# JunzheJosephZhu/DenseMatcher

Measured on AMD Instinct MI355X. Metric: mesh-pairs/sec at N=2048 D=768 k=128, higher is better.
Workload: dtype f16; 1 GPU; configs[1]: batch=64 pairs, N=2048, D=768, k=128 functional-map solve; pairs_per_gpu=64, N=2048, D=768, k=128, basis_dtype=float64, parallelism=pairs sharded over 1 GPU(s), one process per GPU, no data-path collective, process_group_size=1

## Files before the change

### densematcher_amd/csrc/dm_ctx.hip

```cpp
#include <stdarg.h>

#include "dm_internal.h"

int dm_fail(dm_ctx* ctx, int code, const char* fmt, ...) {
    char buf[1024];
    va_list ap;
    va_start(ap, fmt);
    vsnprintf(buf, sizeof(buf), fmt, ap);
    va_end(ap);
    if (ctx) ctx->err = buf;
    return code;
}

static thread_local std::string g_create_err = "null context";

static int create_fail(const char* what, hipError_t e) {
    char buf[512];
    snprintf(buf, sizeof(buf), "dm_create: %s%s%s", what, e != hipSuccess ? ": " : "", e != hipSuccess ? hipGetErrorString(e) : "");
    g_create_err = buf;
    return DM_EHIP;
}

extern "C" int dm_create(int device, void* hip_stream, dm_ctx** out) {
    if (!out) return DM_EINVAL;
// ... 60 lines not shown
    else if (n == "simnn_prio") ctx->opt_simnn_prio = value;
    else if (n == "fit_mfma") ctx->opt_fit_mfma = value;
    else if (n == "solve_pcg") ctx->opt_solve_pcg = value;
    else if (n == "basis_stats") { ctx->opt_basis_stats = value; for (auto& e : ctx->stats) e.valid = false; }
    else if (n == "lsa_reg") ctx->opt_lsa_reg = value;
    else if (n == "p2p_split") ctx->opt_p2p_split = value;
    else if (n == "simnn_persist") ctx->opt_simnn_persist = value;
    else if (n == "p2pfm_direct") ctx->opt_p2pfm_direct = value;
    else if (n == "zoomout_fused") ctx->opt_zoomout_fused = value;
    else if (n == "simnn1_wt") ctx->opt_simnn1_wt = value;
    else if (n == "zoomout_sub_fused") ctx->opt_zoomout_sub_fused = value;
    else if (n == "fps_heat_route") ctx->opt_fps_heat_route = value;
    else if (n == "graph_geod_device") ctx->opt_graph_geod_device = value;
    else if (n == "fmn_eig_route") ctx->opt_fmn_eig_route = value;
    else if (n == "proj_onepass") ctx->opt_proj_onepass = value;
    else return dm_fail(ctx, DM_EINVAL, "dm_set_option: unknown option '%s'", name);
    return DM_OK;
}

extern "C" const char* dm_last_error(const dm_ctx* ctx) { return ctx ? ctx->err.c_str() : g_create_err.c_str(); }
extern "C" const char* dm_version(void) { return DM_VERSION_STRING; }
extern "C" size_t dm_workspace_bytes(const dm_ctx* ctx) { return ctx ? ctx->ws_bytes : 0; }

dm_ctx::basis_stat* dm_stat_entry(dm_ctx* ctx, const void* ptr, int B, int N, int k, int ld, int esz, int n) {
    for (auto& e : ctx->stats)
        if (e.ptr == ptr && e.B == B && e.N == N && e.k == k && e.ld == ld && e.esz == esz && e.n == n && e.buf[0]) return &e;
    dm_ctx::basis_stat& e = ctx->stats[ctx->stats_next];
    ctx->stats_next = (ctx->stats_next + 1) % 4;
    const size_t need = (size_t)B * n * 8;
    if (!e.buf[0] || (size_t)e.B * e.n * 8 < need) {
// ... 131 lines not shown
```

### densematcher_amd/csrc/dm_fmap.hip

```cpp
#include <stdlib.h>

#include "dm_gemm_f64.h"
#include "dm_internal.h"
#include "dm_pcg.h"

struct OutProj {
    float* direct;
    double* partial;
    int B, k, D;
    __device__ __forceinline__ void store(int b, int split, int m, int c, double v) const {
        if (direct) direct[((long long)b * k + m) * D + c] = (float)v;
        else partial[(((long long)split * B + b) * k + m) * D + c] = v;
    }
};

__global__ __launch_bounds__(256) void splitk_reduce_f32_kernel(const double* __restrict__ partial, int nsplit,
                                                                long long n, float* __restrict__ out) {
    const long long i = (long long)blockIdx.x * 256 + threadIdx.x;
    if (i >= n) return;
    double s = 0.0;
    for (int q = 0; q < nsplit; ++q) s += partial[(long long)q * n + i];
    out[i] = (float)s;
}

// ... 887 lines not shown
    DM_REQUIRE(ctx, w_descr >= 0.0 && w_lap >= 0.0 && (w_descr > 0.0 || w_lap > 0.0), "weights must be >= 0 and not both 0");
    DM_CHECK_HIP(ctx, hipSetDevice(ctx->device));
    const size_t bA = (size_t)B * k1 * D * 4, bB = (size_t)B * k2 * D * 4;
    const fmap_solve_plan plan = fmap_solve_plan_for(ctx, B, k1, k2);
    int rc = dm_ws_reserve(ctx, dm_project_f16split_ws(B, N1, D, k1, ld1, (int)sizeof(TR)) + dm_project_f16split_ws(B, N2, D, k2, ld2, (int)sizeof(TR)) +
                                    dm_align_up(bA) + dm_align_up(bB) + dm_align_up((size_t)B * 8) + fmap_solve_ws(plan) + 8192);
    if (rc) return rc;
    double* c00 = (double*)dm_ws_take(ctx, (size_t)B * 8);
    if (!c00) return dm_fail(ctx, DM_ENOMEM, "fmap_fit: workspace not reserved");
    const bool lazy = dm_cdiv(N1, 1024) <= 2 && dm_cdiv(N2, 1024) <= 2;
    float* A = lazy ? nullptr : (float*)dm_ws_take(ctx, bA);
    float* Bm = lazy ? nullptr : (float*)dm_ws_take(ctx, bB);
    if (!lazy && (!A || !Bm)) return dm_fail(ctx, DM_ENOMEM, "fmap_fit: workspace not reserved");
    const float* pA = nullptr; const float* pB = nullptr;
    int nsA = 1, nsB = 1;
    rc = dm_project_f16split_launch<TR>(ctx, B, N1, D, k1, Phi1, ld1, mass1, F1, A, &pA, &nsA);
    if (rc) return rc;
    const dm_c00_args<TR> cz{Phi1, (long long)N1 * ld1, Phi2, (long long)N2 * ld2, mass1, mass2, N1, N2, c00};
    rc = dm_project_f16split_launch<TR>(ctx, B, N2, D, k2, Phi2, ld2, mass2, F2, Bm, &pB, &nsB, &cz);
    if (rc) return rc;
    if (lazy) {
        const long long sA = nsA == 2 ? (long long)B * k1 * D : 0, sB = nsB == 2 ? (long long)B * k2 * D : 0;
        KRowsStackedPart opa{pA, pB, sA, sB, k1, k2, D};
        KRowsPart opb{pA, sA, k1, D};
        return fmap_solve_core(ctx, plan, B, k1, k2, D, opa, opb, lam1, lam2, c00, w_descr, w_lap, C, info);
    }
    KRowsStackedF32 opa{A, Bm, k1, k2, D};
    KRowsF32 opb{A, (long long)k1 * D, D, k1, D};
    return fmap_solve_core(ctx, plan, B, k1, k2, D, opa, opb, lam1, lam2, c00, w_descr, w_lap, C, info);
}
extern "C" int dm_fmap_fit(dm_ctx* ctx, int B, int N1, int N2, int D, int k1, int k2, const float* Phi1, int ld1, const float* Phi2,
                           int ld2, const float* mass1, const float* mass2, const void* F1, const void* F2, const double* lam1,
                           const double* lam2, double w_descr, double w_lap, double* C, int32_t* info) {
    return fmap_fit_impl<float>(ctx, B, N1, N2, D, k1, k2, Phi1, ld1, Phi2, ld2, mass1, mass2, F1, F2, lam1, lam2, w_descr, w_lap, C, info);
// ... 7 lines not shown
```

### densematcher_amd/csrc/dm_internal.h

```cpp
#pragma once

#include <hip/hip_runtime.h>
#include <stdint.h>
#include <stdio.h>
#include <string.h>

#include <string>
#include <unordered_map>
#include <vector>

#include "densematch.h"

#define DM_VERSION_STRING "densematch 0.5.0 (gfx950, abi 7)"

struct dm_ctx {
    int device = 0;
    hipStream_t stream = nullptr;
    std::string err;

    char* ws = nullptr;
    size_t ws_bytes = 0;
    size_t ws_off = 0;

    std::string prof_name;
    std::vector<hipEvent_t> prof_events;
    std::vector<const char*> prof_names;
    std::vector<const char*> prof_syms;
    size_t prof_used = 0;

    std::unordered_map<const void*, size_t> lds_granted;

    int opt_simnn_pipe = 1;
    int opt_knn_split = 1;
    int opt_solve_packed = 0;
    int opt_proj_onepass = 1;
    int opt_fit_mfma = 1;
    int opt_simnn_prio = 0;
    int opt_simnn_big = 0;
    int opt_simnn_band = 4;
    int opt_lsa_reg = 2;
    int opt_solve_pcg = 1;
    int opt_solve_reg = 1;
    int opt_p2p_split = 2;
    int opt_simnn_persist = 1;
    int opt_p2pfm_direct = 1;
    int opt_simnn1_wt = 4;
    int opt_zoomout_fused = 1;
    int opt_zoomout_sub_fused = 1;
    int opt_fps_heat_route = 0;
    int opt_graph_geod_device = 1;
// ... 211 lines not shown
                             int ld2, const float* mass1, const float* A, const float* Bm, const double* lam1, const double* lam2,
                             const double* ops1, const double* ops2, int n_ops, const double* weights, const double* C, double* energy,
                             double* grad, double* keep, bool keep_valid);

int dm_eig_jacobi_sorted(dm_ctx* ctx, int B, int m, double* H, double* V, double* theta, double* Q);

size_t lsa_ws_bytes(int B, int nr, int nc);
int lsa_run(dm_ctx* ctx, int B, int nr, int nc, const double* dense, int n_lr, int KP, const double* E2p, const double* P1p,
            const double* a1p, int maximize, int32_t* col_of_row, int32_t* info);

size_t dm_project_f16split_ws(int B, int N, int D, int k, int ld, int real_bytes);
template <typename TR>
int dm_project_f16split_launch(dm_ctx* ctx, int B, int N, int D, int k, const TR* Phi, int ld, const TR* mass, const void* F,
                               float* Ared, const float** partial_out, int* nsplit_out, const dm_c00_args<TR>* cz = nullptr);
template <typename TR>
int dm_project_f16split(dm_ctx* ctx, int B, int N, int D, int k, const TR* Phi, int ld, const TR* mass,
                        const void* F, float* Ared);
```

### densematcher_amd/csrc/dm_project.hip

```cpp
#include "dm_device.h"
#include "dm_internal.h"

typedef unsigned int u32x4 __attribute__((ext_vector_type(4)));
typedef __fp16 h4_t __attribute__((__vector_size__(4 * sizeof(__fp16))));

constexpr int PT = 128;
constexpr int PTD = 192;
constexpr int PNT = PTD / 64;
constexpr int PFV = PTD / 64;
constexpr int PBK = 32;
constexpr int PLD = 160;
constexpr int PLDF = 224;
constexpr int PSTAGE = 2 * PBK * PLD + PBK * PLDF;

template <int LD>
__device__ __forceinline__ f16x8 tr_frag(const _Float16* base, int row0, int col, int lane) {
    const int t = lane & 15;
    const _Float16* p = base + (row0 + (t >> 2)) * LD + col + 4 * (t & 3);
    const h4_t a = __builtin_amdgcn_ds_read_tr16_b64_v4f16((__attribute__((address_space(3))) h4_t*)p);
    const h4_t b = __builtin_amdgcn_ds_read_tr16_b64_v4f16((__attribute__((address_space(3))) h4_t*)(p + 4 * LD));
    f16x8 r;
    r[0] = (_Float16)a[0]; r[1] = (_Float16)a[1]; r[2] = (_Float16)a[2]; r[3] = (_Float16)a[3];
    r[4] = (_Float16)b[0]; r[5] = (_Float16)b[1]; r[6] = (_Float16)b[2]; r[7] = (_Float16)b[3];
    return r;
// ... 230 lines not shown
        for (int nt = 0; nt < PNT; ++nt)
#pragma unroll
            for (int r = 0; r < 16; ++r) {
                const int m = m0 + wm * 64 + mt * 32 + (r & 3) + 8 * (r >> 2) + 4 * (lane >> 5);
                const int d = d0 + wn * (PTD / 2) + nt * 32 + (lane & 31);
                if (m < p.k && d < p.D) out[(long long)m * p.D + d] = acc[mt][nt][r] * inv_scale;
            }
}

constexpr int P2TD = 384;
constexpr int P2NT = 3;
constexpr int P2LDF = 416;
constexpr int P2STAGE = 2 * PBK * PLD + PBK * P2LDF;
constexpr size_t P2_LDS = (size_t)2 * P2STAGE * sizeof(_Float16) + 16;

template <typename TR>
struct proj2_params {
    const TR* Phi; const TR* mass; const _Float16* F;
    float* partial;
    int B, N, D, k, ld, nsplit, kchunk, tiles_m, tiles_d, ntiles;
    dm_c00_args<TR> cz; int with_c00;
    int flip;
};

template <typename TR, int NMT>
__device__ __forceinline__ void proj2_body(const proj2_params<TR>& p, _Float16* smem, unsigned* slot, int b, int split, int m0, int d0) {
    const int t = threadIdx.x, lane = t & 63, wave = t >> 6;
    const int wm = wave >> 2, wn = wave & 3;
    const int nbeg = split * p.kchunk, nend = min(p.N, nbeg + p.kchunk);
    const TR* Phi = p.Phi + (long long)b * p.N * p.ld;
    const TR* mass = p.mass + (long long)b * p.N;
    const _Float16* F = p.F + (long long)b * p.N * p.D;

    f32x16 acc[NMT > 0 ? NMT : 1][P2NT];
#pragma unroll
    for (int a = 0; a < (NMT > 0 ? NMT : 1); ++a)
#pragma unroll
        for (int c = 0; c < P2NT; ++c)
#pragma unroll
            for (int r = 0; r < 16; ++r) acc[a][c][r] = 0.f;

    const int srow = t >> 4, scol = (t & 15) * 8;
    const int fcol = (t & 15) * (P2TD / 16);
    typedef int i32x4_t __attribute__((ext_vector_type(4)));
    constexpr int NQ = (int)sizeof(TR) / 2;
    const __amdgpu_buffer_rsrc_t rX = __builtin_amdgcn_make_buffer_rsrc(const_cast<TR*>(Phi), (short)0, (int)((unsigned)p.N * p.ld * sizeof(TR)), 0x00020000);
    const __amdgpu_buffer_rsrc_t rM = __builtin_amdgcn_make_buffer_rsrc(const_cast<TR*>(mass), (short)0, (int)((unsigned)p.N * sizeof(TR)), 0x00020000);
    const __amdgpu_buffer_rsrc_t rF = __builtin_amdgcn_make_buffer_rsrc(const_cast<_Float16*>(F), (short)0, (int)((unsigned)p.N * p.D * 2), 0x00020000);
    unsigned colmask = 0;
#pragma unroll
    for (int q = 0; q < 8; ++q) colmask |= (m0 + scol + q < p.k) ? (1u << q) : 0u;
    i32x4_t xrA[NQ], xrB[NQ], anA, anB;
    float xf[8];
    i32x4_t frA[3], frB[3];
#define P2_FENCE() { asm volatile("" ::: "memory"); __builtin_amdgcn_sched_barrier(0); }
#define P2_FETCH_X(s_, xr, an_raw)                                                                            \
    {                                                                                                         \
        const int n_ = nbeg + (s_) * PBK + srow;                                                              \
        const int vo = colmask ? (n_ * p.ld + m0 + scol) * (int)sizeof(TR) : 0x7fffff00;    \
        _Pragma("unroll") for (int q = 0; q < NQ; ++q) xr[q] = __builtin_amdgcn_raw_buffer_load_b128(rX, vo + 16 * q, 0, 0);   \
        if constexpr (sizeof(TR) == 8) {                                                                      \
            const auto m2 = __builtin_amdgcn_raw_buffer_load_b64(rM, n_ * 8, 0, 0);                           \
            an_raw[0] = m2[0]; an_raw[1] = m2[1];                                                             \
        } else {                                                                                              \
            an_raw[0] = __builtin_amdgcn_raw_buffer_load_b32(rM, n_ * 4, 0, 0);                               \
        }                                                                                                     \
        P2_FENCE()                                                                                            \
    }
#define P2_FETCH_F(s_, fr)                                                                                    \
    {                                                                                                         \
        const int n_ = nbeg + (s_) * PBK + srow;                                                              \
        const int vo = (n_ * p.D + d0 + fcol) * 2;                                                            \
        _Pragma("unroll") for (int q = 0; q < 3; ++q) fr[q] = __builtin_amdgcn_raw_buffer_load_b128(rF, vo + 16 * q, 0, 0);   \
        P2_FENCE()                                                                                            \
    }
#define P2_PUBLISH(s_, xr, an_raw)                                                                            \
    {                                                                                                         \
        const bool rv = nbeg + (s_) * PBK + srow < nend;                                                      \
        float an;                                                                                             \
        if constexpr (sizeof(TR) == 8) an = (float)__hiloint2double(an_raw[1], an_raw[0]);                    \
        else an = __int_as_float(an_raw[0]);                                                                  \
        an = rv ? an : 0.f;                                 \
        float mx = 0.f;                                                                                       \
        _Pragma("unroll") for (int q = 0; q < 8; ++q) {                                                       \
            float x_;                                                                                         \
            if constexpr (sizeof(TR) == 8) x_ = (float)__hiloint2double(xr[q >> 1][2 * (q & 1) + 1], xr[q >> 1][2 * (q & 1)]);   \
            else x_ = __int_as_float(xr[q >> 2][q & 3]);                                                      \
            float v_ = x_ * an;                                                                               \
            asm volatile("" : "+v"(v_));                                                                      \
            xf[q] = v_;                                                                                       \
        }                                                                                                     \
        if (colmask != 0xffu && colmask != 0u) {      \
            _Pragma("unroll") for (int q = 0; q < 8; ++q) xf[q] = ((colmask >> q) & 1u) ? xf[q] : 0.f;    \
        }                                                                                                     \
        _Pragma("unroll") for (int q = 0; q < 8; ++q) mx = fmaxf(mx, fabsf(xf[q]));                           \
             \
        mx = fmaxf(mx, __builtin_bit_cast(float, __builtin_amdgcn_update_dpp(0, __builtin_bit_cast(int, mx), 0xB1, 0xF, 0xF, true)));   \
        mx = fmaxf(mx, __builtin_bit_cast(float, __builtin_amdgcn_update_dpp(0, __builtin_bit_cast(int, mx), 0x4E, 0xF, 0xF, true)));   \
        mx = fmaxf(mx, __builtin_bit_cast(float, __builtin_amdgcn_update_dpp(0, __builtin_bit_cast(int, mx), 0x141, 0xF, 0xF, true)));  \
        mx = fmaxf(mx, __builtin_bit_cast(float, __builtin_amdgcn_update_dpp(0, __builtin_bit_cast(int, mx), 0x140, 0xF, 0xF, true)));  \
        const unsigned mu = __builtin_bit_cast(unsigned, mx);                                                 \
        const unsigned m01 = max((unsigned)__builtin_amdgcn_readlane((int)mu, 0), (unsigned)__builtin_amdgcn_readlane((int)mu, 16));   \
        const unsigned m23 = max((unsigned)__builtin_amdgcn_readlane((int)mu, 32), (unsigned)__builtin_amdgcn_readlane((int)mu, 48));  \
        const unsigned mw = max(m01, m23);                                                                    \
        if (lane == 0 && mw != 0u) __hip_atomic_fetch_max(&slot[(s_) % 3], mw, __ATOMIC_RELAXED, __HIP_MEMORY_SCOPE_WORKGROUP);        \
    }
#define P2_STASH(s_, buf_, fr)                                                                                   \
    {                                                                                                         \
        const float smx = __builtin_bit_cast(float, slot[(s_) % 3]);                                          \
        if (smx > run_max) {                                                                                  \
            run_max = smx;                                                                                    \
            int ex = 0;                                                                                       \
            (void)frexpf(smx, &ex);                                                                           \
            const int e2 = min(14 - ex, 100);                                                                 \
            if (e2 < cur_e) {            \
                ratio = ldexpf(1.0f, e2 - cur_e);                                                             \
                cur_e = e2;                                                                                   \
                scale = ldexpf(1.0f, e2);                                                                     \
            }                                                                                                 \
        }                                                                                                     \
        _Float16* Xh = smem + (buf_) * P2STAGE + srow * PLD + scol;                                           \
        _Float16* Xl = Xh + PBK * PLD;                                                                        \
        _Float16* Fs = smem + (buf_) * P2STAGE + 2 * PBK * PLD + srow * P2LDF + fcol;                         \
        f16x8 h, l;                                                                                           \
// ... 7 lines not shown
        *reinterpret_cast<f16x8*>(Xl) = l;                                                                    \
        const bool rvf = nbeg + (s_) * PBK + srow < nend;                                                     \
        _Pragma("unroll") for (int q = 0; q < 3; ++q)                                                         \
            *reinterpret_cast<i32x4_t*>(Fs + 8 * q) = rvf ? fr[q] : i32x4_t{0, 0, 0, 0};                      \
    }

#define P2_RESCALE()                                                                                          \
    if (ratio != 1.0f) {                                                                                      \
        _Pragma("unroll") for (int a = 0; a < (NMT > 0 ? NMT : 1); ++a)                                       \
            _Pragma("unroll") for (int c = 0; c < P2NT; ++c)                                                  \
                _Pragma("unroll") for (int r = 0; r < 16; ++r) acc[a][c][r] *= ratio;                         \
        ratio = 1.0f;                                                                                         \
    }
    float run_max = 0.f, scale = ldexpf(1.0f, 100), ratio = 1.0f;
    int cur_e = 100;
    const int ns = (nend - nbeg + PBK - 1) / PBK;
    if (t < 3) slot[t] = 0u;
    __syncthreads();
    if (ns > 0) {
        P2_FETCH_X(0, xrA, anA)
        P2_FETCH_F(0, frA)
        P2_FETCH_X(1, xrB, anB)
        P2_FETCH_F(1, frB)
        P2_PUBLISH(0, xrA, anA)
        P2_FETCH_X(2, xrA, anA)
    }
    __syncthreads();
    if (ns > 0) {
        P2_STASH(0, 0, frA)
        ratio = 1.0f;
        if (ns > 1) P2_PUBLISH(1, xrB, anB)
    }
    __syncthreads();
#define P2_MMA(buf_)                                                                                          \
        if constexpr (NMT > 0) {                                                                              \
            const _Float16* Xh = smem + (buf_) * P2STAGE;                                                     \
            const _Float16* Xl = Xh + PBK * PLD;                                                              \
            const _Float16* Fs = Xl + PBK * PLD;                                                              \
            _Pragma("unroll") for (int ks = 0; ks < PBK / 16; ++ks) {                                         \
                const int row0 = ks * 16 + 8 * (lane >> 5);                                                   \
                const int sub = 16 * ((lane >> 4) & 1);                \
                f16x8 ah[NMT > 0 ? NMT : 1], al[NMT > 0 ? NMT : 1], bf[P2NT];                                 \
                _Pragma("unroll") for (int x = 0; x < NMT; ++x) {                                             \
                    ah[x] = tr_frag<PLD>(Xh, row0, wm * 64 + x * 32 + sub, lane);                             \
                    al[x] = tr_frag<PLD>(Xl, row0, wm * 64 + x * 32 + sub, lane);                             \
                }                                                                                             \
                _Pragma("unroll") for (int x = 0; x < P2NT; ++x)                                              \
                    bf[x] = tr_frag<P2LDF>(Fs, row0, wn * (P2TD / 4) + x * 32 + sub, lane);                   \
                _Pragma("unroll") for (int mt = 0; mt < NMT; ++mt)                                            \
                    _Pragma("unroll") for (int nt = 0; nt < P2NT; ++nt) {                                     \
                        acc[mt][nt] = __builtin_amdgcn_mfma_f32_32x32x16_f16(ah[mt], bf[nt], acc[mt][nt], 0, 0, 0);   \
                        acc[mt][nt] = __builtin_amdgcn_mfma_f32_32x32x16_f16(al[mt], bf[nt], acc[mt][nt], 0, 0, 0);   \
                    }                                                                                         \
            }                                                                                                 \
        }
#define P2_ITER(s_, XL, ANL, XU, ANU, FL, FU)                                                                 \
    {                                                                                                         \
        const int buf = (s_) & 1;                                                                             \
        P2_FETCH_X((s_) + 3, XL, ANL)                                         \
        P2_FETCH_F((s_) + 2, FL)                                                                              \
        if (p.flip && wave >= 4) {                                                                            \
            if ((s_) + 1 < ns) { P2_STASH((s_) + 1, buf ^ 1, FU) }                                            \
            if ((s_) + 2 < ns) { P2_PUBLISH((s_) + 2, XU, ANU) }                                              \
            __builtin_amdgcn_sched_barrier(0);                                                                \
            P2_MMA(buf)                                                                                       \
        } else {                                                                                              \
            P2_MMA(buf)                                                                                       \
            __builtin_amdgcn_sched_barrier(0);                                                                \
            if ((s_) + 1 < ns) { P2_STASH((s_) + 1, buf ^ 1, FU) }                                            \
            if ((s_) + 2 < ns) { P2_PUBLISH((s_) + 2, XU, ANU) }                                              \
        }                                                                                                     \
        P2_RESCALE()                                                                                          \
        if (t == 0) slot[(s_) % 3] = 0u;                      \
        __syncthreads();                                                                                      \
    }
    for (int s = 0; s < ns; s += 2) {
        P2_ITER(s, xrB, anB, xrA, anA, frA, frB)
        if (s + 1 < ns) P2_ITER(s + 1, xrA, anA, xrB, anB, frB, frA)
    }
#undef P2_ITER
#undef P2_FENCE
#undef P2_MMA
#undef P2_RESCALE
#undef P2_FETCH_X
#undef P2_FETCH_F
#undef P2_PUBLISH
#undef P2_STASH

    if constexpr (NMT > 0) {
        const float inv_scale = 1.0f / scale;
        float* out = p.partial + ((long long)split * p.B + b) * p.k * p.D;
#pragma unroll
        for (int mt = 0; mt < NMT; ++mt)
#pragma unroll
            for (int nt = 0; nt < P2NT; ++nt)
#pragma unroll
                for (int r = 0; r < 16; ++r) {
                    const int m = m0 + wm * 64 + mt * 32 + (r & 3) + 8 * (r >> 2) + 4 * (lane >> 5);
                    const int d = d0 + wn * (P2TD / 4) + nt * 32 + (lane & 31);
                    if (m < p.k && d < p.D) out[(long long)m * p.D + d] = acc[mt][nt][r] * inv_scale;
                }
    }
}

template <typename TR>
__global__ __launch_bounds__(512, 2) void proj_onepass_kernel(proj2_params<TR> p) {
    extern __shared__ __attribute__((aligned(16))) _Float16 smem[];
    const int t = threadIdx.x;
    if ((int)blockIdx.x >= p.ntiles) {
        __shared__ double red[2][4];
        dm_c00_body<TR>(p.cz, (int)blockIdx.x - p.ntiles, t, red);
        return;
    }
    unsigned* slot = reinterpret_cast<unsigned*>(smem + 2 * P2STAGE);
    const int ntile = p.tiles_m * p.tiles_d;
    const int id = xcd_remap(blockIdx.x, p.ntiles);
    const int tile = id % ntile;
    const int split = (id / ntile) % p.nsplit;
    const int b = id / (ntile * p.nsplit);
    const int tm = tile / p.tiles_d, td = tile - tm * p.tiles_d;
    const int m0 = tm * PT, d0 = td * P2TD;
    const int wm = __builtin_amdgcn_readfirstlane(t >> 8);
    const int left = p.k - (m0 + wm * 64);
    if (left > 32) proj2_body<TR, 2>(p, smem, slot, b, split, m0, d0);
    else if (left > 0) proj2_body<TR, 1>(p, smem, slot, b, split, m0, d0);
    else proj2_body<TR, 0>(p, smem, slot, b, split, m0, d0);
}

__global__ __launch_bounds__(256) void proj_reduce_kernel(const float* __restrict__ partial, int nsplit, long long n,
                                                          float* __restrict__ out) {
    const long long i = (long long)blockIdx.x * 256 + threadIdx.x;
    if (i >= n) return;
    double s = 0.0;
    for (int q = 0; q < nsplit; ++q) s += (double)partial[(long long)q * n + i];
    out[i] = (float)s;
}

size_t dm_project_f16split_ws(int B, int N, int D, int k, int ld, int real_bytes) {
    const int nsplit = dm_cdiv(N, 1024);
    return dm_align_up((size_t)nsplit * B * k * D * 4) + dm_align_up((size_t)B * 64 * 4) + 4096 +
           (real_bytes == 8 ? dm_align_up((size_t)B * N * ld * 4) + dm_align_up((size_t)B * N * 4) : 0);
}

template <typename TR>
int dm_project_f16split_launch(dm_ctx* ctx, int B, int N, int D, int k, const TR* Phi, int ld, const TR* mass,
                               const void* F, float* Ared, const float** partial_out, int* nsplit_out, const dm_c00_args<TR>* cz) {
    proj_params<TR> p;
    p.Phi = Phi; p.mass = mass; p.F = (const _Float16*)F;
    p.B = B; p.N = N; p.D = D; p.k = k; p.ld = ld;
    p.tiles_m = dm_cdiv(k, PT); p.tiles_d = dm_cdiv(D, PTD);
    p.kchunk = 1024;
    const int nsplit = dm_cdiv(N, p.kchunk);
    p.nsplit = nsplit;
    if ((long long)N * ld >= (1ll << 31)) return dm_fail(ctx, DM_EINVAL, "dm_project: N * ld must be below 2^31");
    const size_t pbytes = (size_t)nsplit * B * k * D * 4;
    int rc = DM_OK;
    p.partial = (float*)dm_ws_take(ctx, pbytes);
    const int n_part = max(1, min(64, (int)(((long long)N * ld) / 4096)));
    float* amax_part = (float*)dm_ws_take(ctx, (size_t)B * n_part * 4);
    if (!p.partial || !amax_part) return dm_fail(ctx, DM_ENOMEM, "dm_project: workspace not reserved");
    p.amax_part = amax_part; p.n_part = n_part;
    const size_t lds = (size_t)2 * PSTAGE * sizeof(_Float16);
    const bool onepass_ok = (long long)N * ld * (long long)sizeof(TR) < (1ll << 31) - 4096 && (long long)N * D * 2 < (1ll << 31) && (D & 1) == 0 &&
                            (((uintptr_t)F) & 3) == 0;
    if (ctx->opt_proj_onepass && onepass_ok) {
        proj2_params<TR> q;
        q.Phi = Phi; q.mass = mass; q.F = p.F; q.partial = p.partial;
        q.B = B; q.N = N; q.D = D; q.k = k; q.ld = ld; q.nsplit = nsplit; q.kchunk = p.kchunk;
        q.tiles_m = p.tiles_m; q.tiles_d = dm_cdiv(D, P2TD); q.ntiles = q.tiles_m * q.tiles_d * nsplit * B;
        q.with_c00 = cz ? 1 : 0;
        q.flip = 1;
#ifdef DM_EXPERIMENTS
        q.flip = dm_knob("DM_PROJ_FLIP", 1);
#endif
        q.cz = cz ? *cz : dm_c00_args<TR>{};
        rc = dm_grant_lds(ctx, (const void*)proj_onepass_kernel<TR>, P2_LDS);
        if (rc) return rc;
        DM_LAUNCH(ctx, "project_f16split_mfma", proj_onepass_kernel<TR>, dim3(q.ntiles + (cz ? B : 0)), dim3(512), P2_LDS, q);
    } else
    if constexpr (sizeof(TR) == 8) {
        float* phi32 = (float*)dm_ws_take(ctx, (size_t)B * N * ld * 4);
        float* mass32 = (float*)dm_ws_take(ctx, (size_t)B * N * 4);
        if (!phi32 || !mass32) return dm_fail(ctx, DM_ENOMEM, "dm_project: workspace not reserved");
        DM_LAUNCH(ctx, "project_absmax", proj_absmax_kernel<TR>, dim3(n_part + (cz ? 1 : 0), B), dim3(256), 0, Phi, mass, N, ld, k, amax_part, phi32,
                  mass32, n_part, cz ? *cz : dm_c00_args<TR>{});
        proj_params<float> pf;
        pf.Phi = phi32; pf.mass = mass32; pf.F = p.F; pf.amax_part = p.amax_part; pf.n_part = p.n_part; pf.partial = p.partial;
        pf.B = B; pf.N = N; pf.D = D; pf.k = k; pf.ld = ld; pf.nsplit = p.nsplit; pf.kchunk = p.kchunk; pf.tiles_m = p.tiles_m; pf.tiles_d = p.tiles_d;
        rc = dm_grant_lds(ctx, (const void*)proj_f16split_kernel<float>, lds);
        if (rc) return rc;
        DM_LAUNCH(ctx, "project_f16split_mfma", proj_f16split_kernel<float>, dim3(p.tiles_m * p.tiles_d * nsplit * B), dim3(256), lds, pf);
    } else {
        DM_LAUNCH(ctx, "project_absmax", proj_absmax_kernel<TR>, dim3(n_part + (cz ? 1 : 0), B), dim3(256), 0, Phi, mass, N, ld, k, amax_part,
// ... 4 lines not shown
    }
    if (partial_out) *partial_out = p.partial;
    if (nsplit_out) *nsplit_out = nsplit;
    if (Ared) {
        const long long n = (long long)B * k * D;
        DM_LAUNCH(ctx, "project_reduce", proj_reduce_kernel, dim3((unsigned)((n + 255) / 256)), dim3(256), 0, p.partial, nsplit, n,
                  Ared);
    }
    return DM_OK;
}
template int dm_project_f16split_launch<float>(dm_ctx*, int, int, int, int, const float*, int, const float*, const void*, float*, const float**, int*,
                                               const dm_c00_args<float>*);
template int dm_project_f16split_launch<double>(dm_ctx*, int, int, int, int, const double*, int, const double*, const void*, float*, const float**, int*,
                                                const dm_c00_args<double>*);

template <typename TR>
int dm_project_f16split(dm_ctx* ctx, int B, int N, int D, int k, const TR* Phi, int ld, const TR* mass,
                        const void* F, float* Ared) {
    int rc = dm_ws_reserve(ctx, dm_project_f16split_ws(B, N, D, k, ld, (int)sizeof(TR)));
    if (rc) return rc;
    return dm_project_f16split_launch<TR>(ctx, B, N, D, k, Phi, ld, mass, F, Ared, nullptr, nullptr, nullptr);
}
template int dm_project_f16split<float>(dm_ctx*, int, int, int, int, const float*, int, const float*, const void*, float*);
template int dm_project_f16split<double>(dm_ctx*, int, int, int, int, const double*, int, const double*, const void*, float*);
```

### densematcher_amd/engine.py

```python
import ctypes as C
import types

import numpy as np
import torch

from . import _lib
from ._engine_aggre import _AggreOps
from ._engine_dnet import _DiffusionNetOps
from ._engine_eval import _EvalOps
from ._engine_geodesic import GraphTooWide, _GeodesicOps, heat_geodesic_check
from ._engine_jbu import _JbuOps
from ._engine_lift import _LiftOps
from ._engine_mesh import _MeshOps
from ._engine_network import _NetworkOps
from ._engine_render import _RenderOps
from ._engine_vit import _VitOps
from ._operands import fits_abi, host_ptr, ptr as _ptr


class MatchEngine(_MeshOps, _GeodesicOps, _DiffusionNetOps, _LiftOps, _RenderOps, _JbuOps, _AggreOps, _VitOps, _EvalOps, _NetworkOps):
    def __init__(self, device=None, lib_path=None):
        if not torch.cuda.is_available():
            raise RuntimeError("MatchEngine needs a ROCm GPU (gfx950); there is no CPU fallback")
        self.lib = _lib.load(lib_path)
# ... 64 lines not shown
            raise ValueError("matrix contains invalid numeric entries")
        if worst == 1:
            raise ValueError("cost matrix is infeasible")

    def _reals(self, *arrays):
        def dt(a):
            return a.dtype if isinstance(a, torch.Tensor) else getattr(a, "dtype", None)
        f64 = any(a is not None and str(dt(a)).endswith("float64") for a in arrays)
        tdt = torch.float64 if f64 else torch.float32
        return ("_f64" if f64 else "",) + tuple(None if a is None else self._dev(a, tdt, "real") for a in arrays)

    def synchronize(self):
        self.stream.synchronize()

    OPTION_DEFAULTS = {"simnn_pipe": 1, "simnn_persist": 1, "knn_split": 1, "p2p_split": 2, "solve_packed": 0, "solve_reg": 1, "simnn_band": 4, "lsa_reg": 2, "simnn_big": 0,
                       "p2pfm_direct": 1, "zoomout_fused": 1, "proj_onepass": 1, "fit_mfma": 1, "basis_stats": 1, "solve_pcg": 1,
                       "zoomout_sub_fused": 1, "fps_heat_route": 0, "graph_geod_device": 1, "fmn_eig_route": 0}

    def set_option(self, name, value):
        self._chk(self.lib.dm_set_option(self.ctx, name.encode(), int(value)))
        self._options[name] = int(value)

    def get_option(self, name):
        return self._options[name]

    def reset_options(self):
        for k, v in self.OPTION_DEFAULTS.items():
            self.set_option(k, v)

    @staticmethod
    def split_depth(k):
# ... 578 lines not shown
```

Before: 62080 mesh-pairs/s.

## Fuse both mesh projections into one persistent pipelined kernel with cross-tile prefetch

Replaces the two separate one-pass projection launches, one per mesh, with a single persistent kernel sized to the CU count. It walks tiles from both meshes and prefetches the next tile's first stages while the current tile's tail is still computing. This is meant to remove a kernel launch, the tail idle at tile boundaries, and the extra c00 blocks. The price is more register pressure from carrying prefetch state, more complex slot and ring indexing, and a fixed grid that may load-balance worse.

After: 62580 mesh-pairs/s (median of 6 runs). No clear change (+0.8%).

```diff
diff --git a/densematcher_amd/csrc/dm_ctx.hip b/densematcher_amd/csrc/dm_ctx.hip
--- a/densematcher_amd/csrc/dm_ctx.hip
+++ b/densematcher_amd/csrc/dm_ctx.hip
@@ -98,6 +98,7 @@
     else if (n == "graph_geod_device") ctx->opt_graph_geod_device = value;
     else if (n == "fmn_eig_route") ctx->opt_fmn_eig_route = value;
     else if (n == "proj_onepass") ctx->opt_proj_onepass = value;
+    else if (n == "proj_pipeline") ctx->opt_proj_pipeline = value;
     else return dm_fail(ctx, DM_EINVAL, "dm_set_option: unknown option '%s'", name);
     return DM_OK;
 }
diff --git a/densematcher_amd/csrc/dm_fmap.hip b/densematcher_amd/csrc/dm_fmap.hip
--- a/densematcher_amd/csrc/dm_fmap.hip
+++ b/densematcher_amd/csrc/dm_fmap.hip
@@ -925,10 +925,8 @@
     if (!lazy && (!A || !Bm)) return dm_fail(ctx, DM_ENOMEM, "fmap_fit: workspace not reserved");
     const float* pA = nullptr; const float* pB = nullptr;
     int nsA = 1, nsB = 1;
-    rc = dm_project_f16split_launch<TR>(ctx, B, N1, D, k1, Phi1, ld1, mass1, F1, A, &pA, &nsA);
-    if (rc) return rc;
     const dm_c00_args<TR> cz{Phi1, (long long)N1 * ld1, Phi2, (long long)N2 * ld2, mass1, mass2, N1, N2, c00};
-    rc = dm_project_f16split_launch<TR>(ctx, B, N2, D, k2, Phi2, ld2, mass2, F2, Bm, &pB, &nsB, &cz);
+    rc = dm_project_pair_f16split_launch<TR>(ctx, B, D, N1, k1, Phi1, ld1, mass1, F1, A, &pA, &nsA, N2, k2, Phi2, ld2, mass2, F2, Bm, &pB, &nsB, &cz);
     if (rc) return rc;
     if (lazy) {
         const long long sA = nsA == 2 ? (long long)B * k1 * D : 0, sB = nsB == 2 ? (long long)B * k2 * D : 0;
diff --git a/densematcher_amd/csrc/dm_internal.h b/densematcher_amd/csrc/dm_internal.h
--- a/densematcher_amd/csrc/dm_internal.h
+++ b/densematcher_amd/csrc/dm_internal.h
@@ -34,6 +34,7 @@
     int opt_knn_split = 1;
     int opt_solve_packed = 0;
     int opt_proj_onepass = 1;
+    int opt_proj_pipeline = 1;
     int opt_fit_mfma = 1;
     int opt_simnn_prio = 0;
     int opt_simnn_big = 0;
@@ -275,5 +276,9 @@
 int dm_project_f16split_launch(dm_ctx* ctx, int B, int N, int D, int k, const TR* Phi, int ld, const TR* mass, const void* F,
                                float* Ared, const float** partial_out, int* nsplit_out, const dm_c00_args<TR>* cz = nullptr);
 template <typename TR>
+int dm_project_pair_f16split_launch(dm_ctx* ctx, int B, int D, int N1, int k1, const TR* Phi1, int ld1, const TR* mass1, const void* F1, float* Ared1,
+                                    const float** partial1, int* nsplit1, int N2, int k2, const TR* Phi2, int ld2, const TR* mass2, const void* F2,
+                                    float* Ared2, const float** partial2, int* nsplit2, const dm_c00_args<TR>* cz);
+template <typename TR>
 int dm_project_f16split(dm_ctx* ctx, int B, int N, int D, int k, const TR* Phi, int ld, const TR* mass,
                         const void* F, float* Ared);
diff --git a/densematcher_amd/csrc/dm_project.hip b/densematcher_amd/csrc/dm_project.hip
--- a/densematcher_amd/csrc/dm_project.hip
+++ b/densematcher_amd/csrc/dm_project.hip
@@ -268,23 +268,84 @@
 constexpr int P2STAGE = 2 * PBK * PLD + PBK * P2LDF;
 constexpr size_t P2_LDS = (size_t)2 * P2STAGE * sizeof(_Float16) + 16;
 
-template <typename TR>
-struct proj2_params {
+typedef int i32x4_t __attribute__((ext_vector_type(4)));
+
+template <typename TR>
+struct proj2_mesh {
     const TR* Phi; const TR* mass; const _Float16* F;
     float* partial;
-    int B, N, D, k, ld, nsplit, kchunk, tiles_m, tiles_d, ntiles;
+    int N, k, ld, nsplit, tiles_m, tiles_d, ntiles;
+};
+
+template <typename TR>
+struct proj2_params {
+    proj2_mesh<TR> m[2];
+    int B, D, kchunk;
+    int total;
     dm_c00_args<TR> cz; int with_c00;
     int flip;
 };
 
-template <typename TR, int NMT>
-__device__ __forceinline__ void proj2_body(const proj2_params<TR>& p, _Float16* smem, unsigned* slot, int b, int split, int m0, int d0) {
+struct proj2_tile {
+    __amdgpu_buffer_rsrc_t rX, rM, rF;
+    float* out;
+    int nbeg, nend, ns, k, ld, m0, d0;
+};
+struct proj2_src {
+    __amdgpu_buffer_rsrc_t rX, rM, rF;
+    int nbeg, nend, ld, xcol, fcol;
+    unsigned colmask;
+};
+template <typename TR>
+struct proj2_regs {
+    i32x4_t xrA[sizeof(TR) / 2], xrB[sizeof(TR) / 2], anA, anB, frA[3], frB[3];
+    float xf[8];
+};
+
+template <typename TR>
+__device__ __forceinline__ proj2_tile proj2_tile_at(const proj2_params<TR>& p, const proj2_mesh<TR> q, int id) {
+    const int ntile = q.tiles_m * q.tiles_d;
+    const int tile = id % ntile;
+    const int split = (id / ntile) % q.nsplit;
+    const int b = id / (ntile * q.nsplit);
+    const int tm = tile / q.tiles_d, td = tile - tm * q.tiles_d;
+    const TR* Phi = q.Phi + (long long)b * q.N * q.ld;
+    const TR* mass = q.mass + (long long)b * q.N;
+    const _Float16* F = q.F + (long long)b * q.N * p.D;
+    proj2_tile c;
+    c.rX = __builtin_amdgcn_make_buffer_rsrc(const_cast<TR*>(Phi), (short)0, (int)((unsigned)q.N * q.ld * sizeof(TR)), 0x00020000);
+    c.rM = __builtin_amdgcn_make_buffer_rsrc(const_cast<TR*>(mass), (short)0, (int)((unsigned)q.N * sizeof(TR)), 0x00020000);
+    c.rF = __builtin_amdgcn_make_buffer_rsrc(const_cast<_Float16*>(F), (short)0, (int)((unsigned)q.N * p.D * 2), 0x00020000);
+    c.out = q.partial + ((long long)split * p.B + b) * q.k * p.D;
+    c.nbeg = split * p.kchunk;
+    c.nend = min(q.N, c.nbeg + p.kchunk);
+    c.ns = (c.nend - c.nbeg + PBK - 1) / PBK;
+    c.k = q.k; c.ld = q.ld; c.m0 = tm * PT; c.d0 = td * P2TD;
+    return c;
+}
+__device__ __forceinline__ proj2_src proj2_src_of(const proj2_tile& c, int scol, int fcol) {
+    proj2_src s;
+    s.rX = c.rX; s.rM = c.rM; s.rF = c.rF;
+    s.nbeg = c.nbeg; s.nend = c.nend; s.ld = c.ld; s.xcol = c.m0 + scol; s.fcol = c.d0 + fcol;
+    s.colmask = 0;
+#pragma unroll
+    for (int q = 0; q < 8; ++q) s.colmask |= (s.xcol + q < c.k) ? (1u << q) : 0u;
+    return s;
+}
+__device__ __forceinline__ proj2_src proj2_pick(bool first, const proj2_src& a, const proj2_src& b) {
+    proj2_src s;
+    s.rX = first ? a.rX : b.rX; s.rM = first ? a.rM : b.rM; s.rF = first ? a.rF : b.rF;
+    s.nbeg = first ? a.nbeg : b.nbeg; s.nend = first ? a.nend : b.nend; s.ld = first ? a.ld : b.ld;
+    s.xcol = first ? a.xcol : b.xcol; s.fcol = first ? a.fcol : b.fcol; s.colmask = first ? a.colmask : b.colmask;
+    return s;
+}
+
+template <typename TR, int NMT, bool CHAIN>
+__device__ __forceinline__ void proj2_body(const proj2_tile& cur, const proj2_tile& nxt, bool chain, bool primed, int sb, int D, int flip,
+                                           proj2_regs<TR>& rg, _Float16* smem, unsigned* slot) {
     const int t = threadIdx.x, lane = t & 63, wave = t >> 6;
     const int wm = wave >> 2, wn = wave & 3;
-    const int nbeg = split * p.kchunk, nend = min(p.N, nbeg + p.kchunk);
-    const TR* Phi = p.Phi + (long long)b * p.N * p.ld;
-    const TR* mass = p.mass + (long long)b * p.N;
-    const _Float16* F = p.F + (long long)b * p.N * p.D;
+    const int nbeg = cur.nbeg, nend = cur.nend, m0 = cur.m0, d0 = cur.d0;
 
     f32x16 acc[NMT > 0 ? NMT : 1][P2NT];
 #pragma unroll
@@ -296,41 +357,35 @@
 
     const int srow = t >> 4, scol = (t & 15) * 8;
     const int fcol = (t & 15) * (P2TD / 16);
-    typedef int i32x4_t __attribute__((ext_vector_type(4)));
     constexpr int NQ = (int)sizeof(TR) / 2;
-    const __amdgpu_buffer_rsrc_t rX = __builtin_amdgcn_make_buffer_rsrc(const_cast<TR*>(Phi), (short)0, (int)((unsigned)p.N * p.ld * sizeof(TR)), 0x00020000);
-    const __amdgpu_buffer_rsrc_t rM = __builtin_amdgcn_make_buffer_rsrc(const_cast<TR*>(mass), (short)0, (int)((unsigned)p.N * sizeof(TR)), 0x00020000);
-    const __amdgpu_buffer_rsrc_t rF = __builtin_amdgcn_make_buffer_rsrc(const_cast<_Float16*>(F), (short)0, (int)((unsigned)p.N * p.D * 2), 0x00020000);
-    unsigned colmask = 0;
-#pragma unroll
-    for (int q = 0; q < 8; ++q) colmask |= (m0 + scol + q < p.k) ? (1u << q) : 0u;
-    i32x4_t xrA[NQ], xrB[NQ], anA, anB;
-    float xf[8];
-    i32x4_t frA[3], frB[3];
+    const proj2_src cs = proj2_src_of(cur, scol, fcol);
+    const proj2_src nsrc = CHAIN ? proj2_src_of(nxt, scol, fcol) : cs;
+    float (&xf)[8] = rg.xf;
 #define P2_FENCE() { asm volatile("" ::: "memory"); __builtin_amdgcn_sched_barrier(0); }
-#define P2_FETCH_X(s_, xr, an_raw)                                                                            \
+#define P2_FETCH_X(S_, s_, xr, an_raw)                                                                        \
     {                                                                                                         \
-        const int n_ = nbeg + (s_) * PBK + srow;                                                              \
-        const int vo = colmask ? (n_ * p.ld + m0 + scol) * (int)sizeof(TR) : 0x7fffff00;    \
-        _Pragma("unroll") for (int q = 0; q < NQ; ++q) xr[q] = __builtin_amdgcn_raw_buffer_load_b128(rX, vo + 16 * q, 0, 0);   \
+        const int n_ = S_.nbeg + (s_) * PBK + srow;                                                           \
+        const int vo = S_.colmask ? (n_ * S_.ld + S_.xcol) * (int)sizeof(TR) : 0x7fffff00;    \
+        _Pragma("unroll") for (int q = 0; q < NQ; ++q) xr[q] = __builtin_amdgcn_raw_buffer_load_b128(S_.rX, vo + 16 * q, 0, 0);   \
         if constexpr (sizeof(TR) == 8) {                                                                      \
-            const auto m2 = __builtin_amdgcn_raw_buffer_load_b64(rM, n_ * 8, 0, 0);                           \
+            const auto m2 = __builtin_amdgcn_raw_buffer_load_b64(S_.rM, n_ * 8, 0, 0);                        \
             an_raw[0] = m2[0]; an_raw[1] = m2[1];                                                             \
         } else {                                                                                              \
-            an_raw[0] = __builtin_amdgcn_raw_buffer_load_b32(rM, n_ * 4, 0, 0);                               \
+            an_raw[0] = __builtin_amdgcn_raw_buffer_load_b32(S_.rM, n_ * 4, 0, 0);                            \
         }                                                                                                     \
         P2_FENCE()                                                                                            \
     }
-#define P2_FETCH_F(s_, fr)                                                                                    \
+#define P2_FETCH_F(S_, s_, fr)                                                                                \
     {                                                                                                         \
-        const int n_ = nbeg + (s_) * PBK + srow;                                                              \
-        const int vo = (n_ * p.D + d0 + fcol) * 2;                                                            \
-        _Pragma("unroll") for (int q = 0; q < 3; ++q) fr[q] = __builtin_amdgcn_raw_buffer_load_b128(rF, vo + 16 * q, 0, 0);   \
+        const int n_ = S_.nbeg + (s_) * PBK + srow;                                                           \
+        const int vo = (n_ * D + S_.fcol) * 2;                                                                \
+        _Pragma("unroll") for (int q = 0; q < 3; ++q) fr[q] = __builtin_amdgcn_raw_buffer_load_b128(S_.rF, vo + 16 * q, 0, 0);   \
         P2_FENCE()                                                                                            \
     }
-#define P2_PUBLISH(s_, xr, an_raw)                                                                            \
+#define P2_PUBLISH(S_, s_, slot_, xr, an_raw)                                                                 \
     {                                                                                                         \
-        const bool rv = nbeg + (s_) * PBK + srow < nend;                                                      \
+        const unsigned colmask = S_.colmask;                                                                  \
+        const bool rv = S_.nbeg + (s_) * PBK + srow < S_.nend;                                                \
         float an;                                                                                             \
         if constexpr (sizeof(TR) == 8) an = (float)__hiloint2double(an_raw[1], an_raw[0]);                    \
         else an = __int_as_float(an_raw[0]);                                                                  \
@@ -357,11 +412,11 @@
         const unsigned m01 = max((unsigned)__builtin_amdgcn_readlane((int)mu, 0), (unsigned)__builtin_amdgcn_readlane((int)mu, 16));   \
         const unsigned m23 = max((unsigned)__builtin_amdgcn_readlane((int)mu, 32), (unsigned)__builtin_amdgcn_readlane((int)mu, 48));  \
         const unsigned mw = max(m01, m23);                                                                    \
-        if (lane == 0 && mw != 0u) __hip_atomic_fetch_max(&slot[(s_) % 3], mw, __ATOMIC_RELAXED, __HIP_MEMORY_SCOPE_WORKGROUP);        \
+        if (lane == 0 && mw != 0u) __hip_atomic_fetch_max(&slot[slot_], mw, __ATOMIC_RELAXED, __HIP_MEMORY_SCOPE_WORKGROUP);        \
     }
 #define P2_STASH(s_, buf_, fr)                                                                                   \
     {                                                                                                         \
-        const float smx = __builtin_bit_cast(float, slot[(s_) % 3]);                                          \
+        const float smx = __builtin_bit_cast(float, slot[(sb + (s_)) % 3]);                                   \
         if (smx > run_max) {                                                                                  \
             run_max = smx;                                                                                    \
             int ex = 0;                                                                                       \
@@ -399,22 +454,24 @@
     }
     float run_max = 0.f, scale = ldexpf(1.0f, 100), ratio = 1.0f;
     int cur_e = 100;
-    const int ns = (nend - nbeg + PBK - 1) / PBK;
-    if (t < 3) slot[t] = 0u;
+    const int ns = cur.ns;
+    if (!(CHAIN && primed)) {
+        if (t < 3) slot[t] = 0u;
+        __syncthreads();
+        if (ns > 0) {
+            P2_FETCH_X(cs, 0, rg.xrA, rg.anA)
+            P2_FETCH_F(cs, 0, rg.frA)
+            P2_FETCH_X(cs, 1, rg.xrB, rg.anB)
+            P2_FETCH_F(cs, 1, rg.frB)
+            P2_PUBLISH(cs, 0, sb % 3, rg.xrA, rg.anA)
+            P2_FETCH_X(cs, 2, rg.xrA, rg.anA)
+        }
+    }
     __syncthreads();
     if (ns > 0) {
-        P2_FETCH_X(0, xrA, anA)
-        P2_FETCH_F(0, frA)
-        P2_FETCH_X(1, xrB, anB)
-        P2_FETCH_F(1, frB)
-        P2_PUBLISH(0, xrA, anA)
-        P2_FETCH_X(2, xrA, anA)
-    }
-    __syncthreads();
-    if (ns > 0) {
-        P2_STASH(0, 0, frA)
+        P2_STASH(0, 0, rg.frA)
         ratio = 1.0f;
-        if (ns > 1) P2_PUBLISH(1, xrB, anB)
+        if (ns > 1) P2_PUBLISH(cs, 1, (sb + 1) % 3, rg.xrB, rg.anB)
     }
     __syncthreads();
 #define P2_MMA(buf_)                                                                                          \
@@ -442,26 +499,33 @@
 #define P2_ITER(s_, XL, ANL, XU, ANU, FL, FU)                                                                 \
     {                                                                                                         \
         const int buf = (s_) & 1;                                                                             \
-        P2_FETCH_X((s_) + 3, XL, ANL)                                         \
-        P2_FETCH_F((s_) + 2, FL)                                                                              \
-        if (p.flip && wave >= 4) {                                                                            \
+         \
+                                                               \
+        const bool nx3 = CHAIN && chain && (s_) + 3 >= ns, nx2 = CHAIN && chain && (s_) + 2 >= ns;            \
+        const proj2_src sx = CHAIN ? proj2_pick(nx3, nsrc, cs) : cs, sf = CHAIN ? proj2_pick(nx2, nsrc, cs) : cs;   \
+        const int s2 = nx2 ? (s_) + 2 - ns : (s_) + 2;                                                        \
+        const bool pub = (s_) + 2 < ns || (nx2 && (s_) + 2 == ns);                                            \
+        const int pslot = (sb + (s_) + 2) % 3;                                                                \
+        P2_FETCH_X(sx, nx3 ? (s_) + 3 - ns : (s_) + 3, XL, ANL)                                               \
+        P2_FETCH_F(sf, s2, FL)                                                                                \
+        if (flip && wave >= 4) {                                                                              \
             if ((s_) + 1 < ns) { P2_STASH((s_) + 1, buf ^ 1, FU) }                                            \
-            if ((s_) + 2 < ns) { P2_PUBLISH((s_) + 2, XU, ANU) }                                              \
+            if (pub) { P2_PUBLISH(sf, s2, pslot, XU, ANU) }                                                   \
             __builtin_amdgcn_sched_barrier(0);                                                                \
             P2_MMA(buf)                                                                                       \
         } else {                                                                                              \
             P2_MMA(buf)                                                                                       \
             __builtin_amdgcn_sched_barrier(0);                                                                \
             if ((s_) + 1 < ns) { P2_STASH((s_) + 1, buf ^ 1, FU) }                                            \
-            if ((s_) + 2 < ns) { P2_PUBLISH((s_) + 2, XU, ANU) }                                              \
+            if (pub) { P2_PUBLISH(sf, s2, pslot, XU, ANU) }                                                   \
         }                                                                                                     \
         P2_RESCALE()                                                                                          \
-        if (t == 0) slot[(s_) % 3] = 0u;                      \
+        if (t == 0) slot[(sb + (s_)) % 3] = 0u;               \
         __syncthreads();                                                                                      \
     }
     for (int s = 0; s < ns; s += 2) {
-        P2_ITER(s, xrB, anB, xrA, anA, frA, frB)
-        if (s + 1 < ns) P2_ITER(s + 1, xrA, anA, xrB, anB, frB, frA)
+        P2_ITER(s, rg.xrB, rg.anB, rg.xrA, rg.anA, rg.frA, rg.frB)
+        if (s + 1 < ns) P2_ITER(s + 1, rg.xrA, rg.anA, rg.xrB, rg.anB, rg.frB, rg.frA)
     }
 #undef P2_ITER
 #undef P2_FENCE
@@ -474,7 +538,7 @@
 
     if constexpr (NMT > 0) {
         const float inv_scale = 1.0f / scale;
-        float* out = p.partial + ((long long)split * p.B + b) * p.k * p.D;
+        float* out = cur.out;
 #pragma unroll
         for (int mt = 0; mt < NMT; ++mt)
 #pragma unroll
@@ -483,7 +547,7 @@
                 for (int r = 0; r < 16; ++r) {
                     const int m = m0 + wm * 64 + mt * 32 + (r & 3) + 8 * (r >> 2) + 4 * (lane >> 5);
                     const int d = d0 + wn * (P2TD / 4) + nt * 32 + (lane & 31);
-                    if (m < p.k && d < p.D) out[(long long)m * p.D + d] = acc[mt][nt][r] * inv_scale;
+                    if (m < cur.k && d < D) out[(long long)m * D + d] = acc[mt][nt][r] * inv_scale;
                 }
     }
 }
@@ -492,24 +556,62 @@
 __global__ __launch_bounds__(512, 2) void proj_onepass_kernel(proj2_params<TR> p) {
     extern __shared__ __attribute__((aligned(16))) _Float16 smem[];
     const int t = threadIdx.x;
-    if ((int)blockIdx.x >= p.ntiles) {
+    if ((int)blockIdx.x >= p.total) {
         __shared__ double red[2][4];
-        dm_c00_body<TR>(p.cz, (int)blockIdx.x - p.ntiles, t, red);
+        dm_c00_body<TR>(p.cz, (int)blockIdx.x - p.total, t, red);
         return;
     }
     unsigned* slot = reinterpret_cast<unsigned*>(smem + 2 * P2STAGE);
-    const int ntile = p.tiles_m * p.tiles_d;
-    const int id = xcd_remap(blockIdx.x, p.ntiles);
-    const int tile = id % ntile;
-    const int split = (id / ntile) % p.nsplit;
-    const int b = id / (ntile * p.nsplit);
-    const int tm = tile / p.tiles_d, td = tile - tm * p.tiles_d;
-    const int m0 = tm * PT, d0 = td * P2TD;
+    const proj2_tile cur = proj2_tile_at<TR>(p, p.m[0], xcd_remap(blockIdx.x, p.total));
+    proj2_regs<TR> rg;
     const int wm = __builtin_amdgcn_readfirstlane(t >> 8);
-    const int left = p.k - (m0 + wm * 64);
-    if (left > 32) proj2_body<TR, 2>(p, smem, slot, b, split, m0, d0);
-    else if (left > 0) proj2_body<TR, 1>(p, smem, slot, b, split, m0, d0);
-    else proj2_body<TR, 0>(p, smem, slot, b, split, m0, d0);
+    const int left = cur.k - (cur.m0 + wm * 64);
+    if (left > 32) proj2_body<TR, 2, false>(cur, cur, false, false, 0, p.D, p.flip, rg, smem, slot);
+    else if (left > 0) proj2_body<TR, 1, false>(cur, cur, false, false, 0, p.D, p.flip, rg, smem, slot);
+    else proj2_body<TR, 0, false>(cur, cur, false, false, 0, p.D, p.flip, rg, smem, slot);
+}
+
+template <typename TR>
+__device__ __forceinline__ proj2_tile proj2_list_at(const proj2_params<TR>& p, int L) {
+    const proj2_mesh<TR>&m0 = p.m[0], &m1 = p.m[1];
+    const bool first = L < m0.ntiles;
+    proj2_mesh<TR> q;
+    q.Phi = first ? m0.Phi : m1.Phi; q.mass = first ? m0.mass : m1.mass; q.F = first ? m0.F : m1.F; q.partial = first ? m0.partial : m1.partial;
+    q.N = first ? m0.N : m1.N; q.k = first ? m0.k : m1.k; q.ld = first ? m0.ld : m1.ld; q.nsplit = first ? m0.nsplit : m1.nsplit;
+    q.tiles_m = first ? m0.tiles_m : m1.tiles_m; q.tiles_d = first ? m0.tiles_d : m1.tiles_d; q.ntiles = first ? m0.ntiles : m1.ntiles;
+    return proj2_tile_at<TR>(p, q, xcd_remap(first ? L : L - m0.ntiles, q.ntiles));
+}
+
+template <typename TR>
+__global__ __launch_bounds__(512, 2) void proj_pipeline_kernel(proj2_params<TR> p) {
+    extern __shared__ __attribute__((aligned(16))) _Float16 smem[];
+    __shared__ double red[2][4];
+    const int t = threadIdx.x;
+    unsigned* slot = reinterpret_cast<unsigned*>(smem + 2 * P2STAGE);
+    const int wm = __builtin_amdgcn_readfirstlane(t >> 8);
+    const int step = (int)gridDim.x;
+    proj2_regs<TR> rg;
+    bool primed = false;
+    int sb = 0;
+    proj2_tile cur = proj2_list_at<TR>(p, (int)blockIdx.x);
+    for (int L = (int)blockIdx.x; L < p.total; L += step) {
+        const bool more = L + step < p.total;
+        const proj2_tile nxt = proj2_list_at<TR>(p, more ? L + step : L);
+        const bool chain = more && cur.ns >= 4 && (cur.ns & 1) == 0;
+        const int left = cur.k - (cur.m0 + wm * 64);
+        if (left > 32) proj2_body<TR, 2, true>(cur, nxt, chain, primed, sb, p.D, p.flip, rg, smem, slot);
+        else if (left > 0) proj2_body<TR, 1, true>(cur, nxt, chain, primed, sb, p.D, p.flip, rg, smem, slot);
+        else proj2_body<TR, 0, true>(cur, nxt, chain, primed, sb, p.D, p.flip, rg, smem, slot);
+        sb = chain ? (sb + cur.ns) % 3 : 0;
+        primed = chain;
+        cur = nxt;
+    }
+    if (p.with_c00) {
+        for (int b = (int)blockIdx.x; b < p.B; b += step) {
+            dm_c00_body<TR>(p.cz, b, t, red);
+            __syncthreads();
+        }
+    }
 }
 
 __global__ __launch_bounds__(256) void proj_reduce_kernel(const float* __restrict__ partial, int nsplit, long long n,
@@ -528,8 +630,69 @@
 }
 
 template <typename TR>
+static bool proj_onepass_ok(int N, int D, int ld, const void* F) {
+    return (long long)N * ld * (long long)sizeof(TR) < (1ll << 31) - 4096 && (long long)N * D * 2 < (1ll << 31) && (D & 1) == 0 &&
+           (((uintptr_t)F) & 3) == 0;
+}
+template <typename TR>
+static bool proj_pipeline_ok(const dm_ctx* ctx, int N, int D, int ld, const void* F) {
+    return ctx->opt_proj_onepass && ctx->opt_proj_pipeline && proj_onepass_ok<TR>(N, D, ld, F) && (D & 7) == 0 && (((uintptr_t)F) & 15) == 0;
+}
+
+template <typename TR>
+struct proj_job {
+    int N, k, ld; const TR* Phi; const TR* mass; const void* F; float* Ared; const float** partial_out; int* nsplit_out;
+};
+
+template <typename TR>
+static int proj_pipeline_launch(dm_ctx* ctx, int B, int D, int nmesh, const proj_job<TR>* jobs, const dm_c00_args<TR>* cz) {
+    proj2_params<TR> q{};
+    q.B = B; q.D = D; q.kchunk = 1024;
+    for (int i = 0; i < nmesh; ++i) {
+        const proj_job<TR>& j = jobs[i];
+        if ((long long)j.N * j.ld >= (1ll << 31)) return dm_fail(ctx, DM_EINVAL, "dm_project: N * ld must be below 2^31");
+        proj2_mesh<TR>& m = q.m[i];
+        m.Phi = j.Phi; m.mass = j.mass; m.F = (const _Float16*)j.F;
+        m.N = j.N; m.k = j.k; m.ld = j.ld; m.nsplit = dm_cdiv(j.N, q.kchunk);
+        m.tiles_m = dm_cdiv(j.k, PT); m.tiles_d = dm_cdiv(D, P2TD);
+        const long long nt = (long long)m.tiles_m * m.tiles_d * m.nsplit * B;
+        if (nt + q.total >= (1ll << 30)) return dm_fail(ctx, DM_EINVAL, "dm_project: too many tiles");
+        m.ntiles = (int)nt;
+        m.partial = (float*)dm_ws_take(ctx, (size_t)m.nsplit * B * j.k * D * 4);
+        if (!m.partial) return dm_fail(ctx, DM_ENOMEM, "dm_project: workspace not reserved");
+        q.total += m.ntiles;
+    }
+    q.with_c00 = cz ? 1 : 0;
+    q.cz = cz ? *cz : dm_c00_args<TR>{};
+    q.flip = 1;
+#ifdef DM_EXPERIMENTS
+    q.flip = dm_knob("DM_PROJ_FLIP", 1);
+#endif
+    const int ncu = ctx->n_cu >= 8 ? (ctx->n_cu & ~7) : 256;
+    const int grid = q.total <= ncu ? q.total : ncu;
+    int rc = dm_grant_lds(ctx, (const void*)proj_pipeline_kernel<TR>, P2_LDS);
+    if (rc) return rc;
+    DM_LAUNCH(ctx, "project_f16split_mfma", proj_pipeline_kernel<TR>, dim3(grid), dim3(512), P2_LDS, q);
+    for (int i = 0; i < nmesh; ++i) {
+        const proj_job<TR>& j = jobs[i];
+        if (j.partial_out) *j.partial_out = q.m[i].partial;
+        if (j.nsplit_out) *j.nsplit_out = q.m[i].nsplit;
+        if (j.Ared) {
+            const long long n = (long long)B * j.k * D;
+            DM_LAUNCH(ctx, "project_reduce", proj_reduce_kernel, dim3((unsigned)((n + 255) / 256)), dim3(256), 0, q.m[i].partial, q.m[i].nsplit, n,
+                      j.Ared);
+        }
+    }
+    return DM_OK;
+}
+
+template <typename TR>
 int dm_project_f16split_launch(dm_ctx* ctx, int B, int N, int D, int k, const TR* Phi, int ld, const TR* mass,
                                const void* F, float* Ared, const float** partial_out, int* nsplit_out, const dm_c00_args<TR>* cz) {
+    if (proj_pipeline_ok<TR>(ctx, N, D, ld, F)) {
+        const proj_job<TR> job{N, k, ld, Phi, mass, F, Ared, partial_out, nsplit_out};
+        return proj_pipeline_launch<TR>(ctx, B, D, 1, &job, cz);
+    }
     proj_params<TR> p;
     p.Phi = Phi; p.mass = mass; p.F = (const _Float16*)F;
     p.B = B; p.N = N; p.D = D; p.k = k; p.ld = ld;
@@ -546,13 +709,13 @@
     if (!p.partial || !amax_part) return dm_fail(ctx, DM_ENOMEM, "dm_project: workspace not reserved");
     p.amax_part = amax_part; p.n_part = n_part;
     const size_t lds = (size_t)2 * PSTAGE * sizeof(_Float16);
-    const bool onepass_ok = (long long)N * ld * (long long)sizeof(TR) < (1ll << 31) - 4096 && (long long)N * D * 2 < (1ll << 31) && (D & 1) == 0 &&
-                            (((uintptr_t)F) & 3) == 0;
-    if (ctx->opt_proj_onepass && onepass_ok) {
-        proj2_params<TR> q;
-        q.Phi = Phi; q.mass = mass; q.F = p.F; q.partial = p.partial;
-        q.B = B; q.N = N; q.D = D; q.k = k; q.ld = ld; q.nsplit = nsplit; q.kchunk = p.kchunk;
-        q.tiles_m = p.tiles_m; q.tiles_d = dm_cdiv(D, P2TD); q.ntiles = q.tiles_m * q.tiles_d * nsplit * B;
+    if (ctx->opt_proj_onepass && proj_onepass_ok<TR>(N, D, ld, F)) {
+        proj2_params<TR> q{};
+        proj2_mesh<TR>& m = q.m[0];
+        m.Phi = Phi; m.mass = mass; m.F = p.F; m.partial = p.partial;
+        m.N = N; m.k = k; m.ld = ld; m.nsplit = nsplit;
+        m.tiles_m = p.tiles_m; m.tiles_d = dm_cdiv(D, P2TD); m.ntiles = m.tiles_m * m.tiles_d * nsplit * B;
+        q.B = B; q.D = D; q.kchunk = p.kchunk; q.total = m.ntiles;
         q.with_c00 = cz ? 1 : 0;
         q.flip = 1;
 #ifdef DM_EXPERIMENTS
@@ -561,7 +724,7 @@
         q.cz = cz ? *cz : dm_c00_args<TR>{};
         rc = dm_grant_lds(ctx, (const void*)proj_onepass_kernel<TR>, P2_LDS);
         if (rc) return rc;
-        DM_LAUNCH(ctx, "project_f16split_mfma", proj_onepass_kernel<TR>, dim3(q.ntiles + (cz ? B : 0)), dim3(512), P2_LDS, q);
+        DM_LAUNCH(ctx, "project_f16split_mfma", proj_onepass_kernel<TR>, dim3(q.total + (cz ? B : 0)), dim3(512), P2_LDS, q);
     } else
     if constexpr (sizeof(TR) == 8) {
         float* phi32 = (float*)dm_ws_take(ctx, (size_t)B * N * ld * 4);
@@ -596,6 +759,24 @@
 template int dm_project_f16split_launch<double>(dm_ctx*, int, int, int, int, const double*, int, const double*, const void*, float*, const float**, int*,
                                                 const dm_c00_args<double>*);
 
+
+template <typename TR>
+int dm_project_pair_f16split_launch(dm_ctx* ctx, int B, int D, int N1, int k1, const TR* Phi1, int ld1, const TR* mass1, const void* F1, float* Ared1,
+                                    const float** partial1, int* nsplit1, int N2, int k2, const TR* Phi2, int ld2, const TR* mass2, const void* F2,
+                                    float* Ared2, const float** partial2, int* nsplit2, const dm_c00_args<TR>* cz) {
+    if (proj_pipeline_ok<TR>(ctx, N1, D, ld1, F1) && proj_pipeline_ok<TR>(ctx, N2, D, ld2, F2)) {
+        const proj_job<TR> jobs[2] = {{N1, k1, ld1, Phi1, mass1, F1, Ared1, partial1, nsplit1}, {N2, k2, ld2, Phi2, mass2, F2, Ared2, partial2, nsplit2}};
+        return proj_pipeline_launch<TR>(ctx, B, D, 2, jobs, cz);
+    }
+    int rc = dm_project_f16split_launch<TR>(ctx, B, N1, D, k1, Phi1, ld1, mass1, F1, Ared1, partial1, nsplit1, nullptr);
+    if (rc) return rc;
+    return dm_project_f16split_launch<TR>(ctx, B, N2, D, k2, Phi2, ld2, mass2, F2, Ared2, partial2, nsplit2, cz);
+}
+template int dm_project_pair_f16split_launch<float>(dm_ctx*, int, int, int, int, const float*, int, const float*, const void*, float*, const float**, int*,
+                                                    int, int, const float*, int, const float*, const void*, float*, const float**, int*, const dm_c00_args<float>*);
+template int dm_project_pair_f16split_launch<double>(dm_ctx*, int, int, int, int, const double*, int, const double*, const void*, float*, const float**, int*,
+                                                     int, int, const double*, int, const double*, const void*, float*, const float**, int*, const dm_c00_args<double>*);
+
 template <typename TR>
 int dm_project_f16split(dm_ctx* ctx, int B, int N, int D, int k, const TR* Phi, int ld, const TR* mass,
                         const void* F, float* Ared) {
diff --git a/densematcher_amd/engine.py b/densematcher_amd/engine.py
--- a/densematcher_amd/engine.py
+++ b/densematcher_amd/engine.py
@@ -102,7 +102,7 @@
         self.stream.synchronize()
 
     OPTION_DEFAULTS = {"simnn_pipe": 1, "simnn_persist": 1, "knn_split": 1, "p2p_split": 2, "solve_packed": 0, "solve_reg": 1, "simnn_band": 4, "lsa_reg": 2, "simnn_big": 0,
-                       "p2pfm_direct": 1, "zoomout_fused": 1, "proj_onepass": 1, "fit_mfma": 1, "basis_stats": 1, "solve_pcg": 1,
+                       "p2pfm_direct": 1, "zoomout_fused": 1, "proj_onepass": 1, "proj_pipeline": 1, "fit_mfma": 1, "basis_stats": 1, "solve_pcg": 1,
                        "zoomout_sub_fused": 1, "fps_heat_route": 0, "graph_geod_device": 1, "fmn_eig_route": 0}
 
     def set_option(self, name, value):
```
